# pecos/tps

Hardware: AMD Instinct MI355X
Metric: DG RHS evals/sec (MDOF/s) for 3D p=3 reacting cyl at 1/2/4/8 MI355X (higher is better)
Workload: dtype f64

## Files before the change

tps_amd/csrc/kernels.hpp:

```cpp
#ifndef TPSRHS_KERNELS_HPP_
#define TPSRHS_KERNELS_HPP_

#include <hip/hip_runtime.h>

#include <type_traits>

#include "basis.hpp"
#include "physics_dryair.hpp"

namespace tpsrhs {

#ifndef TPSRHS_NO_MFMA
#define TPSRHS_NO_MFMA 0
#endif
#ifndef TPSRHS_LEAN_GENERAL
#define TPSRHS_LEAN_GENERAL 0
#endif
constexpr int cmax(int a, int b) { return a > b ? a : b; }

#ifndef TPSRHS_STAMP
#define TPSRHS_STAMP 0
#endif
#if TPSRHS_STAMP
constexpr int NSTAMP = 16, STAMP_BLOCKS = 1 << 16;
// ... 92 lines not shown
  static constexpr int Q1 = ((DIM_ - 1) + 2 * P_) / 2 + 1 + NC_;
  static constexpr int QV = P_ + 1 + NC_;
  static constexpr int NQV = (DIM_ == 3) ? QV * QV * QV : QV * QV;
  static constexpr int NQ = (DIM_ == 3) ? Q1 * Q1 : Q1;
  static constexpr int NW = (DIM_ == 3) ? Q1 * N1 : 1;
  static constexpr int NFACES = 2 * DIM_;
  static constexpr int NV = 1 << DIM_;
  static constexpr int BLOCK = (NC_ && DIM_ == 3 && P_ >= 2) ? 128 : ((NPE <= 64) ? 64 : ((NPE <= 128) ? 128 : 256));
  static constexpr int EPB = (DIM_ == 3 && NC_) ? (P_ == 3 ? 1 : 2)
                             : (DIM_ == 3 && P_ == 1) ? 3
                             : (DIM_ == 2 && NC_ && P_ == 1) ? 10
                                                             : BLOCK / NPE;
  static constexpr int NODES = EPB * NPE;
  static constexpr int PF = 2 * EPB;
  static constexpr int TN = PF * NF;
  static constexpr int TW = PF * NW;
  static constexpr int TQ = PF * NQ;
  static constexpr int LN = EPB * NF;
  static constexpr int Q_ROUNDS = (TQ + BLOCK - 1) / BLOCK;
  static_assert(DIM_ == 2 || Q_ROUNDS == 1, "3-D: one round of face quadrature points per direction pair");
  static_assert(!(DIM_ == 2 && NC_) || Q_ROUNDS == 1, "2-D Gauss-Lobatto pair: one round per direction pair");
  static constexpr int TQ2 = 2 * TQ;
  static constexpr int Q2_ROUNDS = (TQ2 + BLOCK - 1) / BLOCK;
};

template <class PH, class = void>
struct lean_one_hex : std::false_type {};
template <class PH>
struct lean_one_hex<PH, std::enable_if_t<PH::LEAN_ONE_HEX>> : std::true_type {};
template <class C, class PH>
constexpr bool coulomb_tab() {
  return lean_one_hex<PH>::value && C::DIM == 3 && C::P == 3 && C::NC == 0;
}

template <class C>
struct Tab {
  double x[C::N1], w[C::N1], iw[C::N1], D[C::N1 * C::N1], b0[C::N1], b1[C::N1];
  double xq[C::Q1], wq[C::Q1], B[C::Q1 * C::N1];
  double xv[C::QV], wv[C::QV];
};

struct ForcingDev {
  int has_pg, nheat, nsponge, pad;
  double pg[3];
  struct Heat {
    double value, radius, len;
    double p1[3], axis[3];
  } heat[TPSRHS_MAXHEATSOURCES];
  struct Sponge {
    int type, pad;
    double normal[3], p0[3], pinit[3];
    double r1, r2, mult;
    double target[TPSRHS_MAXEQUATIONS];
    int mixed_out, n_plane;
    const int *plane_nodes;
    double *msum;
  } sponge[TPSRHS_MAXSPONGEZONES];
  const double *joule;
  int nps, pad2;
  struct Scalar {
    double x0[3], radius, value;
  } ps[TPSRHS_MAXPASSIVESCALARS];
};

struct RkDev {
  int mode, sp_first, sp_last, pad;
// ... 1408 lines not shown
      const double val = lean1_point<C>(Wb, k, bq, ll);
      if (k >= 1 && k <= NVEL)
        gv[(k - 1) + CD * DIM] = val;
      else if (CD == 0)
        gn[k] = 0.0 + n[CD] * val;
      else
        gn[k] += n[CD] * val;
    }
#pragma unroll
    for (int k = 0; k < NEQ; k++) {
      if (k >= 1 && k <= NVEL)
        asm volatile("" : "+v"(gv[(k - 1) + CD * DIM]));
      else
        asm volatile("" : "+v"(gn[k]));
    }
    block_sync<C::BLOCK>();
  };
  stage(std::integral_constant<int, 0>());
  stage(std::integral_constant<int, 1>());
  stage(std::integral_constant<int, 2>());
}
template <class C, class PH, int D>
__device__ inline void lean1_state_dir(const double *sU, double *Tb, double *Wb, const Tab<C> &tab, const Tables1D &ct0, double *u,
                                       const LeanLane<C> &ll) {
  const Tables1D &ct = fresh_table(ct0);
  lean1_lines<C, D, PH::NEQ>(sU, Tb, Wb, ct, ll, ll.template trace_src<D>());
  double bq[C::N1];
#pragma unroll
  for (int a = 0; a < C::N1; a++) bq[a] = tab.B[ll.pb + a];
#pragma unroll
  for (int k = 0; k < PH::NEQ; k++) u[k] = lean1_point<C>(Wb, k, bq, ll);
  block_sync<C::BLOCK>();
}
template <class C, class PH>
__device__ inline void visc_phase_lean1(const MeshDev &m, const int2 *sFI, typename PH::PRef prm0, int e0, const double *sU,
                                        const double *gradUp_q, bool node_on0, double *sJ, double *Tb, double *Wb,
                                        const double *sV, const Tab<C> &tab, const Tables1D &ct, double *__restrict__ TB,
                                        int tid0 STAMP_PARAM) {
  constexpr int NEQ = PH::NEQ, DIM = C::DIM;
  static_assert(DIM == 3 && C::Q_ROUNDS == 1 && PH::NVEL == 3 && C::BLOCK == 64 && C::EPB == 1, "3-D, one wave = one hex");
  const bool node_on = __builtin_amdgcn_readfirstlane(node_on0) != 0;
#pragma clang loop unroll(disable)
  for (int d = 0; d < DIM; d++) {
    typename PH::PRef prm = PH::relaunder(prm0);
    int tid = tid0;
    asm volatile("" : "+v"(tid));
    const int pf = tid / C::NQ, q = tid - pf * C::NQ;
    const int le = pf >> 1, s = pf & 1;
    const bool on = tid < C::TQ && (e0 + le) < m.ne;
    int nb = 0;
    double n[DIM] = {1.0, 0.0, 0.0};
    if (on) {
      double wq, Xq[DIM];
      nb = sFI[le * C::NFACES + 2 * d + s].x;
      face_geometry_rt<C>(d, &sV[le * C::NV * DIM], tab, s, q, n, wq, Xq);
    }
    const int np_lane = on ? PH::visc_passes(prm, nb) : 0;
    const int npass = (__ballot(np_lane == 2) != 0) ? 2 : ((__ballot(np_lane >= 1) != 0) ? 1 : 0);
    double *out = TB + static_cast<int64_t>((e0 + le) * C::NFACES + 2 * d + s) * ((NEQ - 1) * C::NQ) + q;
    if (on && np_lane == 0) {
#pragma unroll
      for (int eq = 1; eq < NEQ; eq++) out[(eq - 1) * C::NQ] = 0.0;
    }
#pragma clang loop unroll(disable)
    for (int pass = 0; pass < npass; pass++) {
      double u[NEQ];
      int tid1 = tid0;
      asm volatile("" : "+v"(tid1));
      const LeanLane<C> ll(static_cast<unsigned>(tid1) & (C::BLOCK - 1));
      if (d == 0)
        lean1_state_dir<C, PH, 0>(sU, Tb, Wb, tab, ct, u, ll);
      else if (d == 1)
        lean1_state_dir<C, PH, 1>(sU, Tb, Wb, tab, ct, u, ll);
      else
        lean1_state_dir<C, PH, 2>(sU, Tb, Wb, tab, ct, u, ll);
      STAMP(5);
      PH::clamp_species(u);
      double gnext[NEQ];
      unsigned long long ga = lean1_grad_base<C>(gradUp_q, e0);
      const unsigned long long gstep = static_cast<unsigned long long>(m.ndofs) * sizeof(double);
      if (node_on) {
        lean1_issue_grad<NEQ>(ga, gstep, ll.lane, gnext);
      } else {
#pragma unroll
        for (int eq = 0; eq < NEQ; eq++) gnext[eq] = 0.0;
      }
      typename PH::ViscLean cf;
      if (pass < np_lane) {
        typename PH::PRef pq = PH::relaunder(prm);
        double Us[NEQ];
        typename PH::WallFlux w;
        PH::visc_pass_state(pq, nb, pass, u, n, Us, w);
        if constexpr (coulomb_tab<C, PH>())
          PH::template visc_point_lean<true>(pq, Us, w, cf);
        else
          PH::visc_point_lean(pq, Us, w, cf);
      }
      STAMP(6);
      double gv[DIM * DIM], gn[NEQ];
      if (d == 0)
        lean1_grad_dir<C, PH, 0>(ga, gstep, node_on, gnext, sJ, Tb, Wb, tab, ct, n, gv, gn, ll);
      else if (d == 1)
        lean1_grad_dir<C, PH, 1>(ga, gstep, node_on, gnext, sJ, Tb, Wb, tab, ct, n, gv, gn, ll);
      else
        lean1_grad_dir<C, PH, 2>(ga, gstep, node_on, gnext, sJ, Tb, Wb, tab, ct, n, gv, gn, ll);
      STAMP(7);
      if (pass < np_lane) {
        double f[NEQ];
        PH::visc_normal_flux_lean(cf, gv, gn, n, f);
        if (nb >= 0) {
#pragma unroll
          for (int eq = 1; eq < NEQ; eq++) out[(eq - 1) * C::NQ] = f[eq];
        } else if (pass == 0) {
#pragma unroll
          for (int eq = 1; eq < NEQ; eq++) out[(eq - 1) * C::NQ] = -0.5 * f[eq];
        } else {
#pragma unroll
          for (int eq = 1; eq < NEQ; eq++) out[(eq - 1) * C::NQ] -= 0.5 * f[eq];
        }
      }
      STAMP(8);
    }
  }
}
template <class C, class PH>
__device__ inline void visc_phase_2d(const MeshDev &m, const int2 *sFI, typename PH::PRef prm, int e0,
// ... 209 lines not shown
  jump(std::integral_constant<int, 1>());
  if (DIM == 3) {
    trace_lines<C, (DIM == 3 ? 2 : 0), NEQ>(sUp, sJ, ct, tid);
    block_sync<C::BLOCK>();
    store_neighbour_traces<C, NEQ>(ta2, sJ, sJ + NEQ * C::TN, tid);
    block_sync<C::BLOCK>();
    jump(std::integral_constant<int, (DIM == 3 ? 2 : 0)>());
  }
  if constexpr (C::NC) {
    if constexpr (C::NPE == 64 && C::BLOCK == 128 && !TPSRHS_NO_MFMA) {
      static_assert(L::V >= 64 * 17, "LDS buffer of the MFMA inverse mass");
      nc_apply_minv_mfma<C, NEQ * DIM>(m.minv, pool + L::O_V, node_on, e0, nd, tid, g);
    }
    else
      nc_apply_minv<C, NEQ * DIM>(m.minv, pool + L::O_V, node_on, e0 + le_n, le_n, nd, tid, g);
  }

  STAMP(3);
  if (node_on) {
    const unsigned n = static_cast<unsigned>(e0 + le_n) * C::NPE + nd;
#pragma unroll
    for (int k = 0; k < NEQ * DIM; k++) field_ptr(gradUp, k, m.ndofs)[n] = g[k];
    if constexpr (L::G_IN_LDS) {
#pragma unroll
      for (int k = 0; k < NEQ * DIM; k++) sJ[k * C::NODES + tid] = g[k];
    }
  }
  if (L::G_IN_LDS) block_sync<C::BLOCK>();
  STAMP(4);
  if constexpr (L::LEAN3D) {
    asm volatile("s_waitcnt vmcnt(0)" ::: "memory");
    const double *gq = gradUp;
    const unsigned node = static_cast<unsigned>(e0 + le_n) * C::NPE + nd;
    if constexpr (PH::LEAN_ONE_HEX && C::EPB == 1 && C::BLOCK % C::LN == 0 && !TPSRHS_LEAN_GENERAL)
      visc_phase_lean1<C, PH>(m, sFI, prm, e0, sU, gq, node_on, sJ, sUp, sW, sV, tab, ct, TB, tid STAMP_ARG);
    else
      visc_phase_lean3d<C, PH>(m, sFI, prm, e0, sU, gq, node_on, node, sJ, sUp, sW, sV, tab, ct, TB, tid STAMP_ARG);
    STAMP_FLUSH();
    return;
  }

  if constexpr (DIM == 2) {
    if constexpr (PH::HEAVY) {
      __shared__ double sDist[C::NODES];
      const bool ml_on = m.ml.distance != nullptr;
      if (ml_on) {
        if (tid < C::NODES)
          sDist[tid] = node_on ? m.ml.distance[static_cast<int64_t>(e0 + le_n) * C::NPE + nd] : 0.0;
        block_sync<C::BLOCK>();
      }
      visc_phase_2d<C, PH>(m, sFI, prm, e0, sU, g, node_on, sJ, sUp, sV, tab, ct, TB, tid, ml_on ? sDist : nullptr);
    } else {
      visc_phase_2d<C, PH>(m, sFI, prm, e0, sU, g, node_on, sJ, sUp, sV, tab, ct, TB, tid);
    }
  } else if constexpr (PH::TWO_STEP && C::Q_ROUNDS == 1) {
    visc_phase_heavy3d<C, PH>(m, sFI, prm, e0, sU, sJ, sUp, sW, sV, tab, ct, TB, tid STAMP_ARG);
  } else if constexpr (PH::HEAVY) {
#pragma clang loop unroll(disable)
    for (int d = 0; d < DIM; d++) {
      double v[C::Q_ROUNDS][L::NVF];
      if (d == 0)
        visc_interp_dir<C, PH, 0>(sU, g, node_on, sJ, sUp, sW, tab, ct, v, tid);
      else if (d == 1)
        visc_interp_dir<C, PH, 1>(sU, g, node_on, sJ, sUp, sW, tab, ct, v, tid);
      else
        visc_interp_dir<C, PH, (DIM == 3 ? 2 : 0)>(sU, g, node_on, sJ, sUp, sW, tab, ct, v, tid);
      visc_points<C, PH>(m, sFI, prm, e0, d, v, sV, tab, TB, tid);
    }
  } else {
// ... 573 lines not shown
  }
  if (node_on) {
#pragma unroll
    for (int eq = 0; eq < NEQ; eq++) sU[eq * C::NODES + tid] = u[eq];
  }
  block_sync<C::BLOCK>();
  FSTAMP(1);

  double inv_mass = 0.0, speed = 0.0;
  double src[NEQ];
#pragma unroll
  for (int eq = 0; eq < NEQ; eq++) src[eq] = 0.0;
  if (node_on) {
    double F[NEQ * DIM];
    double radius = 1.0;
    double Xn[DIM] = {};
    if constexpr (PH::AXISYM || (PH::HEAVY && DIM == 2)) {
      if (PH::AXISYM || m.vs.enabled) {
        double xi[DIM];
#pragma unroll
        for (int d = 0; d < DIM; d++) xi[d] = tab.x[idx[d]];
        position<DIM>(&sV[le_n * C::NV * DIM], xi, Xn);
      }
      if (PH::AXISYM) radius = Xn[0];
    }
    {
      double uc[NEQ];
#pragma unroll
      for (int eq = 0; eq < NEQ; eq++) uc[eq] = u[eq];
      PH::clamp_species(uc);
      const typename PH::State st = PH::make_state(prm, uc);
      speed = PH::max_char_speed(prm, uc, st);
      typename PH::FluxCoef fc;
      if constexpr (coulomb_tab<C, PH>())
        PH::template flux_coeffs<true>(prm, uc, st, fc);
      else if constexpr (PH::TWO_STEP)
        PH::flux_coeffs(prm, uc, st, fc);
      if (PH::HAS_SOURCE) {
        double up[NEQ];
        PH::prim(prm, u, up);
        PH::source(prm, u, up, gr, src);
        if constexpr (PH::AXISYM) PH::axisym_source(prm, u, up, gr, radius, src);
      }

      if constexpr (PH::HEAVY && DIM == 2) {
        const bool ml_on = m.ml.distance != nullptr;
        __shared__ double sVsw[C::BLOCK];
        const EddyCtx ec = closure_ctx(m, true, ml_on ? m.ml.distance[static_cast<int64_t>(e0 + le_n) * C::NPE + nd] : 0.0, Xn, sVsw);
        if constexpr (PH::TWO_STEP)
          PH::total_flux(prm, uc, st, fc, gr, PH::AXISYM ? radius : -1.0, F, ec);
        else
          PH::total_flux(prm, uc, st, gr, radius, F, ec);
      } else if constexpr (PH::TWO_STEP)
        PH::total_flux(prm, uc, st, fc, gr, PH::AXISYM ? radius : -1.0, F);
      else if constexpr (PH::AXISYM)
        PH::total_flux(prm, uc, st, gr, radius, F);
      else if constexpr (PH::LES) {
        PointCtx pc;
        double xn[DIM];
#pragma unroll
        for (int d = 0; d < DIM; d++) xn[d] = tab.x[idx[d]];
        position<DIM>(&sV[le_n * C::NV * DIM], xn, pc.X);
        pc.delta = prm.elem_delta[e0 + le_n];
        PH::total_flux(prm, uc, st, gr, F, &pc);
      } else
        PH::total_flux(prm, uc, st, gr, F);
    }
// ... 323 lines not shown
```

tps_amd/csrc/physics_plasma.hpp:

```cpp
#ifndef TPSRHS_PHYSICS_PLASMA_HPP_
#define TPSRHS_PHYSICS_PLASMA_HPP_

#include <hip/hip_runtime.h>

#include "physics_dryair.hpp"
#if __has_include("coulomb_table.hpp")
#include "coulomb_table.hpp"
#define TPSRHS_HAVE_COULOMB_TABLE 1
#endif

namespace tpsrhs {

#pragma clang fp reciprocal(on)

constexpr double kRgas = 8.3144598;
constexpr double kAvogadro = 6.0221409e+23;
constexpr double kBoltz = kRgas / kAvogadro;
constexpr double kEps0 = 8.8541878128e-12;
constexpr double kQe = 1.60218e-19;
constexpr double kMolarQe = kQe * kAvogadro;
constexpr double kPi = 3.14159265358979323846;
constexpr double kXeps = 1.0e-30;

struct TableDev {
// ... 3 lines not shown
};
struct ChemDev {
  int num_reactions, electron_index;
  double min_temperature;
  double energy[TPSRHS_MAXREACTIONS];
  double rate[TPSRHS_MAXCHEMPARAMS * TPSRHS_MAXREACTIONS];
  double keq[TPSRHS_MAXCHEMPARAMS * TPSRHS_MAXREACTIONS];
  signed char reactant[TPSRHS_MAXSPECIES * TPSRHS_MAXREACTIONS];
  signed char product[TPSRHS_MAXSPECIES * TPSRHS_MAXREACTIONS];
  signed char model[TPSRHS_MAXREACTIONS];
  signed char detailed_balance[TPSRHS_MAXREACTIONS];
  TableDev table[TPSRHS_MAXREACTIONS];
  signed char table_share[TPSRHS_MAXREACTIONS];
  int radiation;
  TableDev nec;
};

constexpr int PLASMA_MAXBC = 8;
template <int NSP>
struct PlasmaParams {
  double mw[NSP], charge[NSP], eform[NSP], cv[NSP], cp[NSP];
  double imw[NSP], mwp[NSP], sq_mwp[NSP], kf_imwp[NSP], sq_muw_idfc[NSP * NSP];
  double vf_sq_mwp[NSP], ke_fac, ke_fac3, qkb_charge[NSP], rg_imw[NSP], icv_e;
  double c_visc, c_bulk, c_k, c_ke, c_diff[NSP], c_mtfreq[NSP];
  int c_eidx;
  int third_order, multiply;
  int coll[NSP * NSP];
  int cmask_diag, cmask_e, cmask_h;
  double mult_flux[4], mult_spcs, mult_diff, mult_mobil;
  const ChemDev *chem;
  int eq_system, use_bc_in_grad, num_bcs, axisymmetric;
  BcDev bc[PLASMA_MAXBC];
  const double *ctab;
};

__device__ inline double ipow(double x, int k) {
  double r = 1.0;
  for (int i = 0; i < k; i++) r *= x;
  return r;
}
template <class TD>
__device__ inline int table_interval(const TD &t, double xe) {
  if (t.inv_dx > 0.0) {
    int g = static_cast<int>((xe - t.x0) * t.inv_dx);
    g = max(0, min(t.n - 2, g));
    if (g > 0 && !(xe > t.x[g])) g--;
    if (g < t.n - 2 && xe > t.x[g + 1]) g++;
    if ((g == 0 || xe > t.x[g]) && (g == t.n - 2 || !(xe > t.x[g + 1]))) return g;
  }
  int count = t.n, first = 0;
  while (count > 0) {
    int it = first;
    const int step = count / 2;
    it += step;
    if (xe > t.x[it]) {
      first = ++it;
      count -= step + 1;
    } else {
      count = step;
    }
  }
  first = max(1, min(t.n - 1, first));
  return first - 1;
}
template <class TD>
__device__ inline double table_eval(const TD &t, double xe) {
// ... 82 lines not shown
  for (int r = 0; r < NUNI; r++) {
    if (todo) {
      const int u = __builtin_amdgcn_readfirstlane(idx);
      if (idx == u) {
        coulomb::horner<NF>(ctab + u * coulomb::STRIDE, t, g);
        todo = false;
      }
    }
  }
  if (todo) coulomb::horner<NF>(tab + idx * coulomb::STRIDE, t, g);
}
template <int NF>
__device__ inline void cfit_tab(const double *tab, const Arg &a, double (&out)[NF]) {
  static_assert(NF == 2 || NF == 8, "att11 and rep22, or all eight");
  const bool on = tab != nullptr && coulomb::in_range(a.ln);
  if (on) {
    ctab_eval<NF, TPSRHS_COULOMB_UNIFORM>(tab, a.ln, true, out);
#pragma unroll
    for (int f = 0; f < NF; f++) out[f] *= a.inv2;
  } else if constexpr (NF == 8) {
    double A[4], B[4];
    cfit_n<4>(kFitA, a, A);
    cfit_n<4>(kFitB, a, B);
#pragma unroll
    for (int f = 0; f < 4; f++) {
      out[f] = A[f];
      out[4 + f] = B[f];
    }
  } else {
    out[0] = att11(a);
    out[1] = rep22(a);
  }
}
#endif
__constant__ static double c_coulomb[2][2][5][4] = {
    {{{0.2150, 5.2194, 1.0472, 1.2435}, {0.0991, 7.4684, 1.0155, 1.1536}, {0.0616, 7.8271, 0.9452, 1.1105},
      {0.0308, 13.9567, 0.9511, 1.1803}, {0.0232, 13.7888, 0.9148, 1.1532}},
     {{0, 0, 0, 0}, {0.2423, 4.6796, 1.3290, 1.1279}, {0.1221, 8.7542, 1.3875, 1.1110}, {0.0619, 18.2538, 1.4341, 1.1618},
      {0, 0, 0, 0}}},
    {{{0.3904, 0.9100, 1.1025, 1.0544}, {0.1547, 1.6597, 1.1725, 0.9792}, {0.0814, 2.5815, 1.1948, 0.9570},
      {0.0683, 1.9774, 1.2033, 0.8264}, {0.0346, 4.5177, 1.2132, 0.9294}},
     {{0, 0, 0, 0}, {0.4128, 1.2436, 1.1830, 1.0123}, {0.2203, 1.8832, 1.2059, 0.9851}, {0.1323, 2.7248, 1.2129, 0.9847},
      {0, 0, 0, 0}}}};
__device__ inline double ArAr11(double lnT) { return 2.2910e-18 * fexp(-0.3032 * lnT); }
__device__ inline double ArAr22(double T) { return 1.7e-18 * fast_rsqrt(fast_sqrt(T)); }
__device__ inline double iArAr22(double sqrtT) { return fast_sqrt(sqrtT) * (1.0 / 1.7e-18); }
__device__ inline double ArAr1P11(double lnT) { return 4.574321e-18 * fexp(-0.1805 * lnT); }
__device__ inline double eAr1r(int r, double logT) {
  const double C[5][9] = {
      {6.36254140e-18, 1.84835040e-18, -5.87727093e-18, 3.20023027e-18, -8.50509054e-19, 1.28163820e-19,
       -1.11712910e-20, 5.25649382e-22, -1.03296658e-23},
      {1.91338172e-17, 5.45418129e-18, -1.78361685e-17, 9.75657946e-18, -2.61115722e-18, 3.98310268e-19,
       -3.53503678e-20, 1.70375066e-21, -3.45211955e-23},
      {3.04685398e-17, 8.39750994e-18, -2.88132528e-17, 1.60147037e-17, -4.34837891e-18, 6.73136845e-19,
       -6.06704580e-20, 2.97216168e-21, -6.12760944e-23},
      {3.90777949e-17, 1.04696956e-17, -3.73774204e-17, 2.10610498e-17, -5.79029566e-18, 9.07573157e-19,
       -8.28466766e-20, 4.11188110e-21, -8.59225098e-23},
      {4.41333290e-17, 1.15696010e-17, -4.25651305e-17, 2.42442440e-17, -6.73359258e-18, 1.06641697e-18,
       -9.83933863e-20, 4.93775812e-21, -1.04362372e-22}};
  double fit = C[r - 1][0] * fast_rcp(logT), pw = 1.0;
#pragma unroll
  for (int k = 1; k < 9; k++) {
    fit += C[r - 1][k] * pw;
    pw *= logT;
  }
  return fit;
// ... 24 lines not shown
  }
}
}

#ifndef TPSRHS_PLASMA_MINW_FLUX
#define TPSRHS_PLASMA_MINW_FLUX 2
#endif
#ifndef TPSRHS_PLASMA_MINW_GRAD3
#define TPSRHS_PLASMA_MINW_GRAD3 2
#endif
#ifndef TPSRHS_PLASMA_MINW_GRAD_LEAN
#define TPSRHS_PLASMA_MINW_GRAD_LEAN 3
#endif
enum { TRANSPORT_CONSTANT = 0, TRANSPORT_ARGON_MINIMAL = 1, TRANSPORT_ARGON_MIXTURE = 2 };

template <int DIM_, int NVEL_, int NSP_, bool AMBI, bool TWOT, int TRANSPORT>
struct PlasmaPhys {
  static constexpr int DIM = DIM_, NVEL = NVEL_, NSP = NSP_;
  static constexpr int NACTIVE = AMBI ? NSP_ - 2 : NSP_ - 1;
  static constexpr int NEQ = NVEL_ + 2 + NACTIVE + (TWOT ? 1 : 0);
  static constexpr int IE = NSP_ - 2, IB = NSP_ - 1;
  static constexpr int ITH = NVEL_ + 1, ITE = NEQ - 1;
  static constexpr bool HAS_SOURCE = true;
  static constexpr bool TWO_TEMPERATURE = TWOT;
  static constexpr int MAX_ORDER = 4;
  static constexpr bool HAS_NR_BC = false;
  static constexpr bool LES = false;
  static constexpr bool HAS_MIXED_OUT = false;
  static constexpr bool VISC_USES_GRAD_RHO = true;
  static constexpr bool AXISYM = NVEL_ > DIM_;
  static constexpr int MINW_GRAD = (NSP_ > 3) ? 1 : TPSRHS_PLASMA_MINW_GRAD3;
  static constexpr bool LEAN_TRACE = (NSP_ == 3) && (DIM_ == 3);
  static constexpr bool LEAN_ONE_HEX = LEAN_TRACE && !TWOT && TRANSPORT == TRANSPORT_ARGON_MINIMAL;
  static constexpr bool LAUNDER_FLUX = false;
  static constexpr int minw_grad(int dim, int p, int nc) {
    return (LEAN_TRACE && dim == 3 && !nc && p <= 3) ? TPSRHS_PLASMA_MINW_GRAD_LEAN : MINW_GRAD;
  }
  static constexpr int MINW_FLUX = (NSP_ > 6 || (NSP_ > 3 && DIM_ == 3)) ? 1 : TPSRHS_PLASMA_MINW_FLUX;
  typedef PlasmaParams<NSP_> Params;
  typedef const Params *KArg;
  typedef const Params __attribute__((address_space(4))) &PRef;
  typedef const BcDev __attribute__((address_space(4))) &BcRef;
  __device__ static inline PRef pref(KArg k) { return *(const Params __attribute__((address_space(4))) *)k; }
  __device__ static inline PRef relaunder(PRef p) {
    const unsigned long long a = reinterpret_cast<unsigned long long>(&p);
    unsigned lo = __builtin_amdgcn_readfirstlane(static_cast<unsigned>(a));
    unsigned hi = __builtin_amdgcn_readfirstlane(static_cast<unsigned>(a >> 32));
    asm volatile("" : "+s"(lo), "+s"(hi));
    return *reinterpret_cast<const Params __attribute__((address_space(4))) *>((static_cast<unsigned long long>(hi) << 32) | lo);
  }
  struct Transport {};

  struct State {
    double ir, k, p, pe, Th, Te, c;
    double vel[NVEL];
    double n[NSP];
  };

  __device__ static inline void number_densities(PRef p, const double *U, double *n) {
#pragma unroll
    for (int sp = 0; sp < NSP; sp++) n[sp] = 0.0;
#pragma unroll
    for (int sp = 0; sp < NACTIVE; sp++) n[sp] = U[NVEL + 2 + sp] * p.imw[sp];
    double rhoB = U[0];
#pragma unroll
    for (int sp = 0; sp < NACTIVE; sp++) rhoB -= p.mw[sp] * n[sp];
// ... 215 lines not shown
    double att, rep, ar1p, are, arar;
  };
  template <int L, int R>
  __device__ static inline CollTab coll_table(int mask, bool with_e, const MixColl &c) {
    CollTab t;
    t.att = t.rep = t.ar1p = t.are = t.arar = 0.0;
    const coll::Arg &a = with_e ? c.e : c.h;
    const double ln = with_e ? c.lnTe : c.lnTh;
    if (mask & (1 << TPSRHS_CLMB_ATT)) {
      const double *k = coll::c_coulomb[0][L - 1][R - 1];
      t.att = c.circle * coll::cfit(k[0], k[1], k[2], k[3], a);
    }
    if (mask & (1 << TPSRHS_CLMB_REP)) {
      const double *k = coll::c_coulomb[1][L - 1][R - 1];
      t.rep = c.circle * coll::cfit(k[0], k[1], k[2], k[3], a);
    }
    if (mask & (1 << TPSRHS_AR_AR1P)) t.ar1p = coll::ArAr1P11(ln);
    if (mask & (1 << TPSRHS_AR_E)) t.are = coll::eAr1r(R, ln);
    if (mask & (1 << TPSRHS_AR_AR)) t.arar = (L == 1) ? coll::ArAr11(ln) : coll::ArAr22(c.Th);
    return t;
  }
  __device__ static inline double coll_pick(PRef p, int i, int j, const CollTab &t) {
    const int a = i < j ? i : j, b = i < j ? j : i;
    const int type = p.coll[a + b * NSP];
    const double q_att = t.att, q_rep = t.rep, q_ar1p = t.ar1p, q_are = t.are, q_arar = t.arar;
    double v = q_arar;
    v = (type == TPSRHS_AR_E) ? q_are : v;
    v = (type == TPSRHS_AR_AR1P) ? q_ar1p : v;
    v = (type == TPSRHS_CLMB_REP) ? q_rep : v;
    v = (type == TPSRHS_CLMB_ATT) ? q_att : v;
    return v;
  }

  template <bool CTAB = false>
  __device__ static inline void transport_coeffs(PRef p, const double *U, double Th, double Te, bool diffusion,
                                                 TCoef &t) {
#ifndef TPSRHS_HAVE_COULOMB_TABLE
    static_assert(!CTAB, "coulomb_table.hpp is not part of this build");
#endif
    static_assert(!CTAB || (!TWOT && TRANSPORT == TRANSPORT_ARGON_MINIMAL), "the table serves the single-temperature argon-minimal closure");
    const Species q = species(p, U);
#pragma unroll
    for (int sp = 0; sp < NSP; sp++) {
      t.n[sp] = q.n[sp];
      t.Y[sp] = q.Y[sp];
      t.dX[sp] = t.mob[sp] = 0.0;
    }
    t.intot = q.intot;
    t.imho = 0.0;
    double diff[NSP] = {}, mob[NSP] = {};
    const double iTe = fast_rcp(Te), iTh = TWOT ? fast_rcp(Th) : iTe;
    if (TRANSPORT == TRANSPORT_CONSTANT) {
      t.visc = p.c_visc;
      t.bulk = p.c_bulk;
      t.k = p.c_k;
      t.ke = p.c_ke;
#pragma unroll
      for (int sp = 0; sp < NSP; sp++) {
        diff[sp] = p.c_diff[sp];
        const double itemp = (sp == p.c_eidx) ? iTe : iTh;
        mob[sp] = p.qkb_charge[sp] * itemp * diff[sp];
      }
    } else if (TRANSPORT == TRANSPORT_ARGON_MIXTURE) {
      const MixColl c = mix_inputs(p, q.n, Th, Te);
      const double sTe = fast_sqrt(Te), sTh = TWOT ? fast_sqrt(Th) : sTe;
      t.visc = t.bulk = t.k = 0.0;
      {
        const CollTab d22 = coll_table<2, 2>(p.cmask_diag, false, c);
#pragma unroll
        for (int sp = 0; sp < NSP; sp++) {
          if (sp == IE) continue;
          const double sv = p.vf_sq_mwp[sp] * sTh * fast_rcp(coll_pick(p, sp, sp, d22));
// ... 39 lines not shown
            ibd[i + j * NSP] = ibd[j + i * NSP] = ((i == IE || j == IE) ? nrsTe : nrsTh) * p.sq_muw_idfc[i + j * NSP] *
                                                  coll_pick(p, i, j, (i == IE || j == IE) ? pe : ph);
#pragma unroll
        for (int i = 0; i < NSP; i++) {
          double a = 0.0;
#pragma unroll
          for (int j = 0; j < NSP; j++)
            if (i != j) a += (q.X[j] + kXeps) * ibd[i + j * NSP];
          diff[i] = (1.0 - q.Y[i]) * fast_rcp(a);
          mob[i] = p.qkb_charge[i] * ((i == IE) ? iTe : iTh) * diff[i];
        }
      }
      if (p.multiply) {
        t.visc *= p.mult_flux[0];
        t.bulk *= p.mult_flux[1];
        t.k *= p.mult_flux[2];
        t.ke *= p.mult_flux[3];
#pragma unroll
        for (int sp = 0; sp < NSP; sp++) {
          diff[sp] *= p.mult_diff;
          mob[sp] *= p.mult_mobil;
        }
      }
    } else {
      const double sTe = fast_sqrt(Te), sTh = TWOT ? fast_sqrt(Th) : sTe;
      const Debye d = debye(q.n, Th, Te, iTh, iTe);
      const double lnTe = flog(Te), lnTh = TWOT ? flog(Th) : lnTe;
      double QeAr, Qatt, rep22h;
      if (p.third_order) {
        double A[4], B[4], QN[5];
#ifdef TPSRHS_HAVE_COULOMB_TABLE
        if constexpr (CTAB) {
          double g[8];
          coll::cfit_tab<8>(p.ctab, d.e, g);
#pragma unroll
          for (int f = 0; f < 4; f++) {
            A[f] = g[f];
            B[f] = g[4 + f];
          }
        } else
#endif
        {
          coll::cfit_n<4>(coll::kFitA, d.e, A);
          coll::cfit_n<4>(coll::kFitB, d.e, B);
        }
        coll::eAr1r_n<5>(lnTe, QN);
        Qatt = A[0] * d.circle;
        QeAr = QN[0];
        const double Q2[3] = {d.circle * A[1], d.circle * A[2], d.circle * A[3]};
        const double QI[5] = {Qatt, d.circle * B[0], d.circle * B[1], d.circle * B[2], d.circle * B[3]};
        rep22h = TWOT ? coll::rep22(d.h) * d.circle : Q2[0];
        t.ke = third_order_ke(q.X, Q2, QI, QN, sTe, p.ke_fac3);
      } else {
        QeAr = coll::eAr1r(1, lnTe);
#ifdef TPSRHS_HAVE_COULOMB_TABLE
        if constexpr (CTAB) {
          double g[2];
          coll::cfit_tab<2>(p.ctab, d.e, g);
          Qatt = g[0] * d.circle;
          rep22h = g[1] * d.circle;
        } else
#endif
        {
          Qatt = coll::att11(d.e) * d.circle;
          rep22h = coll::rep22(d.h) * d.circle;
        }
        t.ke = p.ke_fac * sTe * q.X[I_E] * fast_rcp(TWOT ? coll::rep22(d.e) * d.circle : rep22h);
      }
      const double sv_ion = p.vf_sq_mwp[I_ION] * sTh * fast_rcp(rep22h);
      const double sv_n = p.vf_sq_mwp[I_N] * sTh * coll::iArAr22(sTh);
      t.bulk = 0.0;
      t.visc = q.X[I_ION] * sv_ion + q.X[I_N] * sv_n;
      t.k = q.X[I_ION] * (sv_ion * p.kf_imwp[I_ION]) + q.X[I_N] * (sv_n * p.kf_imwp[I_N]);
      __builtin_amdgcn_sched_barrier(0);
      if (diffusion) {
        const double nrsTe = q.ntot * (sTe * iTe), nrsTh = TWOT ? q.ntot * (sTh * iTh) : nrsTe;
        double ibd[NSP * NSP];
#pragma unroll
        for (int i = 0; i < NSP * NSP; i++) ibd[i] = 0.0;
        ibd[I_E + I_N * NSP] = ibd[I_N + I_E * NSP] = nrsTe * p.sq_muw_idfc[I_E + I_N * NSP] * QeAr;
        ibd[I_N + I_ION * NSP] = ibd[I_ION + I_N * NSP] = nrsTh * p.sq_muw_idfc[I_N + I_ION * NSP] * coll::ArAr1P11(lnTh);
        ibd[I_E + I_ION * NSP] = ibd[I_ION + I_E * NSP] = nrsTe * p.sq_muw_idfc[I_E + I_ION * NSP] * Qatt;
#pragma unroll
        for (int i = 0; i < NSP; i++) {
          double a = 0.0;
#pragma unroll
          for (int j = 0; j < NSP; j++)
            if (i != j) a += (q.X[j] + kXeps) * ibd[i + j * NSP];
          diff[i] = (1.0 - q.Y[i]) * fast_rcp(a);
          mob[i] = p.qkb_charge[i] * ((i == I_E) ? iTe : iTh) * diff[i];
        }
// ... 178 lines not shown
#pragma unroll
    for (int i = 0; i < DIM; i++) divV += g[(1 + i) + i * NEQ];
    double tau_t[DIM] = {};
    if (AXISYM) {
      if (radius > 0) divV += s.vel[0] / radius;
      double ttr = g[3 + 0 * NEQ];
      if (radius > 0) ttr -= s.vel[2] / radius;
      tau_t[0] = ttr * t.visc;
      tau_t[1] = t.visc * g[3 + 1 * NEQ];
    }
#pragma unroll
    for (int i = 0; i < DIM; i++) {
      double vt = 0.0;
#pragma unroll
      for (int j = 0; j < DIM; j++) {
        double st = t.visc * (g[(1 + j) + i * NEQ] + g[(1 + i) + j * NEQ]);
        if (i == j) st += bulk * divV;
        Fv[(1 + j) + i * NEQ] = st;
        vt += st * s.vel[j];
      }
      if (AXISYM) {
        Fv[(1 + 2) + i * NEQ] = tau_t[i];
        vt += s.vel[2] * tau_t[i];
      }
      double e = vt + k * g[ITH + i * NEQ];
#pragma unroll
      for (int sp = 0; sp < NSP; sp++) e -= h[sp] * t.V[sp + i * NSP];
      Fv[ITH + i * NEQ] += e;
#pragma unroll
      for (int sp = 0; sp < NACTIVE; sp++) Fv[(NVEL + 2 + sp) + i * NEQ] = -U[NVEL + 2 + sp] * t.V[sp + i * NSP];
    }
  }
  typedef TCoef FluxCoef;
  template <bool CTAB = false>
  __device__ static inline void flux_coeffs(PRef p, const double *U, const State &s, FluxCoef &c) {
    if (p.eq_system == TPSRHS_EULER) return;
    transport_coeffs<CTAB>(p, U, s.Th, s.Te, true, c);
  }
  __device__ static inline void total_flux(PRef p, const double *U, const State &s, const FluxCoef &c,
                                           const double *g, double radius, double *F, const EddyCtx &ec = eddy_off()) {
    double Fv[NEQ * DIM];
    visc_flux(p, U, s, c, g, radius, Fv, ec);
    const double H = U[ITH] + s.p;
#pragma unroll
    for (int d = 0; d < DIM; d++) {
      F[0 + d * NEQ] = U[1 + d] - Fv[0 + d * NEQ];
#pragma unroll
      for (int i = 0; i < NVEL; i++) F[1 + i + d * NEQ] = U[1 + i] * s.vel[d] + (i == d ? s.p : 0.0) - Fv[1 + i + d * NEQ];
      F[ITH + d * NEQ] = s.vel[d] * H - Fv[ITH + d * NEQ];
#pragma unroll
      for (int sp = 0; sp < NACTIVE; sp++)
        F[(NVEL + 2 + sp) + d * NEQ] = U[NVEL + 2 + sp] * s.vel[d] - Fv[(NVEL + 2 + sp) + d * NEQ];
      if (TWOT) F[ITE + d * NEQ] = (U[ITE] + s.pe) * s.vel[d] - Fv[ITE + d * NEQ];
    }
  }
  struct WallFlux {
    bool species, heavy_heat, electron_heat;
    double Vn[NSP], hf, ef, nm;
  };
  __device__ static inline WallFlux no_prescription() {
    WallFlux w;
    w.species = w.heavy_heat = w.electron_heat = false;
#pragma unroll
    for (int sp = 0; sp < NSP; sp++) w.Vn[sp] = 0.0;
    w.hf = w.ef = 0.0;
    w.nm = 1.0;
    return w;
  }
  __device__ static inline void visc_normal_flux(PRef p, const double *U, const double *g, const double *n,
                                                 double radius, const WallFlux &w, double *Fn, const EddyCtx &ec = eddy_off()) {
// ... 324 lines not shown
      Fn[1 + i] = sn;
      e += sn * c.vel[i];
    }
    double HF = 0.0, EF = 0.0;
    if (w.heavy_heat) {
      HF = w.hf * w.nm;
    } else {
      const double k = TWOT ? c.t.k : c.t.k + c.t.ke;
      HF -= k * gn[ITH];
#pragma unroll
      for (int sp = 0; sp < NSP; sp++)
        if (!(TWOT && sp == IE)) HF += c.h[sp] * Vn[sp];
    }
    if (TWOT) {
      if (w.electron_heat) {
        EF = w.ef * w.nm;
      } else {
        EF -= c.t.ke * gn[ITE];
        EF += c.h[IE] * Vn[IE];
      }
    }
    Fn[ITH] = e - HF - EF;
#pragma unroll
    for (int sp = 0; sp < NACTIVE; sp++) Fn[NVEL + 2 + sp] = -U[NVEL + 2 + sp] * Vn[sp];
    if (TWOT) Fn[ITE] = -EF;
  }
  static constexpr int NIN = 1 + NACTIVE;
  struct ViscLean {
    double mu, bulkp, kq, ke;
    double vel[NVEL];
    double hf0, ef0, sf0[NACTIVE];
    double hfc[NIN], efc[NIN], sfc[NACTIVE][NIN];
  };
  template <bool CTAB = false>
  __device__ static inline void visc_point_lean(PRef p, const double *U, const WallFlux &w, ViscLean &L) {
    const State s = make_state(p, U);
    TCoef t;
    transport_coeffs<CTAB>(p, U, s.Th, s.Te, !w.species, t);
    double h[NSP];
    enthalpies(p, s, h);
    L.mu = t.visc;
    L.bulkp = t.bulk - 2. / 3. * t.visc;
#pragma unroll
    for (int d = 0; d < NVEL; d++) L.vel[d] = s.vel[d];
    L.kq = w.heavy_heat ? 0.0 : (TWOT ? t.k : t.k + t.ke);
    L.hf0 = w.heavy_heat ? w.hf * w.nm : 0.0;
    L.ke = (TWOT && !w.electron_heat) ? t.ke : 0.0;
    L.ef0 = (TWOT && w.electron_heat) ? w.ef * w.nm : 0.0;
#pragma unroll
    for (int sp = 0; sp < NACTIVE; sp++) L.sf0[sp] = 0.0;
#pragma unroll
    for (int j = 0; j < NIN; j++) {
      L.hfc[j] = L.efc[j] = 0.0;
#pragma unroll
      for (int sp = 0; sp < NACTIVE; sp++) L.sfc[sp][j] = 0.0;
    }
    if (w.species) {
      double Vn[NSP];
#pragma unroll
      for (int sp = 0; sp < NSP; sp++) Vn[sp] = w.Vn[sp] * w.nm;
      if (!w.heavy_heat) {
#pragma unroll
        for (int sp = 0; sp < NSP; sp++)
          if (!(TWOT && sp == IE)) L.hf0 += h[sp] * Vn[sp];
      }
      if (TWOT && !w.electron_heat) L.ef0 += h[IE] * Vn[IE];
#pragma unroll
      for (int sp = 0; sp < NACTIVE; sp++) L.sf0[sp] = -U[NVEL + 2 + sp] * Vn[sp];
    } else {
#pragma unroll
      for (int j = 0; j < NIN; j++) {
// ... 373 lines not shown
```

tps_amd/csrc/tpsrhs.hip:

```cpp
#include "operator.hpp"
#include "element_geometry.hpp"
#include "integrals.hpp"
#include "locate_device.hpp"
#include "operator_plan.hpp"
#include "physics_dryair.hpp"
#include "physics_dryair_axisym.hpp"
#include "physics_plasma.hpp"
#include "plasma_params_host.hpp"
#include "point_locate.hpp"
#include "record_log.hpp"
#include "sampling.hpp"
#include "statistics.hpp"
#include "time_integrators.hpp"
#include "wall_distance.hpp"
#include "wall_faces.hpp"

#include <dlfcn.h>

#include <cmath>
#include <map>
#include <mutex>
#include <new>
#include <thread>
#include <type_traits>
// ... 68 lines not shown
    std::vector<double> t(coulomb::SIZE);
    coll::coulomb_table_fill(t.data());
    return t;
  }();
  return table;
}

template <int NSP>
void fill_plasma_params(tpsrhs_operator *op, const tpsrhs_disc *disc, const tpsrhs_physics *phys, int num_bcs,
                        const tpsrhs_bc *bcs) {
  static_assert(sizeof(PlasmaParams<NSP>) <= sizeof(op->params), "parameter block too large");
  PlasmaParams<NSP> &p = *new (op->params) PlasmaParams<NSP>;
  std::unique_ptr<ChemDev> c(new ChemDev);
  try {
    tpsrhs::fill_plasma_params<NSP>(p, *c, disc, phys, num_bcs, bcs, [op](const tpsrhs_table &t) { return upload_table(op, t); });
  } catch (const UnsupportedConfig &e) {
    throw Unsupported(e.what());
  }
  op->d_chem = DevBuf<ChemDev>(1);
  p.chem = static_cast<ChemDev *>(op->d_chem.get());
  HIP_CHECK(hipMemcpy(op->d_chem.get(), c.get(), sizeof(ChemDev), hipMemcpyHostToDevice));
}

void fill_mixture_params(tpsrhs_operator *op, const OperatorPlan &pl, const tpsrhs_disc *disc, const tpsrhs_physics *phys,
                         int num_bcs, const tpsrhs_bc *bcs) {
  switch (phys->mixture.num_species) {
    case 3:
      fill_plasma_params<3>(op, disc, phys, num_bcs, bcs);
      if (pl.coulomb_table) {
        const char *env = std::getenv("TPSRHS_COULOMB_TABLE");
        if (!env || env[0] != '0') {
          op->d_coulomb = DevBuf<double>(coulomb_table_host());
          reinterpret_cast<PlasmaParams<3> *>(op->params)->ctab = op->d_coulomb.get();
        }
      }
      break;
    case 4: fill_plasma_params<4>(op, disc, phys, num_bcs, bcs); break;
    case 5: fill_plasma_params<5>(op, disc, phys, num_bcs, bcs); break;
    case 6: fill_plasma_params<6>(op, disc, phys, num_bcs, bcs); break;
    case 7: fill_plasma_params<7>(op, disc, phys, num_bcs, bcs); break;
    default: fill_plasma_params<8>(op, disc, phys, num_bcs, bcs); break;
  }
  char msg[512] = {0};
  const int rc = load_family(pl.unit)(op, phys->mixture.two_temperature ? 1 : 0, pl.transport, msg, static_cast<int>(sizeof msg));
  if (rc == TPSRHS_ERR_UNSUPPORTED) throw Unsupported(msg);
  if (rc == TPSRHS_ERR_INVALID_ARGUMENT) throw std::invalid_argument(msg);
  if (rc != TPSRHS_OK) throw DeviceError(msg);
}

void upload_lte_tables(tpsrhs_operator *op, LteParams *lp, const tpsrhs_physics *phys) {
  const tpsrhs_lte &in = phys->lte;
  lp->tab_e = upload_table(op, in.energy_table);
  lp->tab_R = upload_table(op, in.gas_constant_table);
  lp->tab_c = upload_table(op, in.sound_speed_table);
  tpsrhs_table rev = in.energy_table;
  rev.x_data = in.energy_table.f_data;
  rev.f_data = in.energy_table.x_data;
  lp->tab_T = upload_table(op, rev);
  {
    const int N = in.energy_table.n_data, nh = 4 * (N - 1);
    const double *ex = in.energy_table.f_data;
    const double de = (ex[N - 1] - ex[0]) / nh;
    std::vector<int> hint(nh);
    int idx = 0;
    for (int j = 0; j < nh; j++) {
      const double left = ex[0] + j * de;
// ... 851 lines not shown
int tpsrhs_math_eval(int function, int64_t n, const double *x, double *y) {
  if (function < 0 || function > 6 || n < 0 || !x || !y) return fail(TPSRHS_ERR_INVALID_ARGUMENT, "math_eval");
  return guarded([&] {
    int ndev = 0;
    if (hipGetDeviceCount(&ndev) != hipSuccess || ndev == 0) throw std::runtime_error("no HIP device visible");
    if (n > 0) {
      hipLaunchKernelGGL(k_math_eval, dim3(static_cast<unsigned>((n + 255) / 256)), dim3(256), 0, nullptr, function, n, x, y);
      HIP_CHECK(hipGetLastError());
    }
    HIP_CHECK(hipDeviceSynchronize());
  });
}

namespace {
__global__ void k_coulomb_eval(int route, const double *tab, int64_t n, const double *__restrict__ x, double *__restrict__ out) {
  const int64_t i = static_cast<int64_t>(blockIdx.x) * 256 + threadIdx.x;
  if (i >= n) return;
  coll::Arg a;
  a.ln = x[i];
  a.inv2 = 1.0;
  double g[8];
  if (route == 0 || !coulomb::in_range(a.ln)) {
    coll::cfit_tab<8>(nullptr, a, g);
  } else if (route == 1) {
    coll::ctab_eval<8, 2>(tab, a.ln, true, g);
  } else {
    coll::ctab_eval<8, 0>(tab, a.ln, true, g);
  }
#pragma unroll
  for (int f = 0; f < 8; f++) out[f * n + i] = g[f];
}
}

int tpsrhs_coulomb_eval(int route, int64_t n, const double *x, double *out) {
  if (route < 0 || route > 2 || n < 0 || !x || !out) return fail(TPSRHS_ERR_INVALID_ARGUMENT, "coulomb_eval");
  return guarded([&] {
    int ndev = 0;
    if (hipGetDeviceCount(&ndev) != hipSuccess || ndev == 0) throw std::runtime_error("no HIP device visible");
    DevBuf<double> tab(coulomb_table_host());
    if (n > 0) {
      hipLaunchKernelGGL(k_coulomb_eval, dim3(static_cast<unsigned>((n + 255) / 256)), dim3(256), 0, nullptr, route, tab.get(), n, x, out);
      HIP_CHECK(hipGetLastError());
    }
    HIP_CHECK(hipDeviceSynchronize());
  });
}

int tpsrhs_table_eval(const tpsrhs_table *table, int64_t n, const double *x, double *f) {
  if (!table || n < 0 || !x || !f) return fail(TPSRHS_ERR_INVALID_ARGUMENT, "table_eval");
  return guarded([&] {
    int ndev = 0;
    if (hipGetDeviceCount(&ndev) != hipSuccess || ndev == 0) throw std::runtime_error("no HIP device visible");
    tpsrhs_operator tmp;
    (void)hipGetDevice(&tmp.device);
    const TableDev td = upload_table(&tmp, *table);
    if (n > 0) {
      hipLaunchKernelGGL(k_table_eval, dim3(static_cast<unsigned>((n + 255) / 256)), dim3(256), 0, nullptr, td, n, x, f);
      HIP_CHECK(hipGetLastError());
    }
    HIP_CHECK(hipDeviceSynchronize());
  });
}

int tpsrhs_mult_times(tpsrhs_handle h, int capacity, double *milliseconds) {
  if (!h || h->sets_recorded == 0 || !milliseconds) return 0;
  if (hipStreamSynchronize(h->stream) != hipSuccess) return 0;
  const int nsets = static_cast<int>(std::min<int64_t>(h->sets_recorded, tpsrhs_operator::MAXSETS));
  int n = 0;
  for (; n < nsets && n < capacity; n++) {
    float ms = 0.f;
    if (hipEventElapsedTime(&ms, h->evs[n][0], h->evs[n][NKERN]) != hipSuccess) return n;
    milliseconds[n] = ms;
  }
// ... 950 lines not shown
```

Before: 13170.

## Stage Coulomb table intervals in a per-wave LDS window for transport evaluation

```diff
diff --git a/tps_amd/csrc/coulomb_probe.hip b/tps_amd/csrc/coulomb_probe.hip
--- /dev/null
+++ b/tps_amd/csrc/coulomb_probe.hip
@@ -0,0 +1,36 @@
+#include <hip/hip_runtime.h>
+
+#include <algorithm>
+#include <cstdint>
+
+#include "physics_plasma.hpp"
+
+using namespace tpsrhs;
+
+namespace {
+constexpr int COULOMB_PROBE_BLOCKS = 4;
+__global__ __launch_bounds__(64) void k_coulomb_eval_window(const double *tab, int64_t n, const double *__restrict__ x,
+                                                            double *__restrict__ out) {
+  typedef coll::Window<TPSRHS_COULOMB_WINDOW_W> Win;
+  __shared__ __attribute__((aligned(16))) double mem[Win::DOUBLES];
+  Win win;
+  win.create(mem, true);
+  for (int64_t c0 = static_cast<int64_t>(blockIdx.x) * 64; c0 < n; c0 += static_cast<int64_t>(gridDim.x) * 64) {
+    const int64_t i = c0 + threadIdx.x;
+    if (i < n) {
+      coll::Arg a;
+      a.ln = x[i];
+      a.inv2 = 1.0;
+      double g[8];
+      coll::cfit_tab<8>(tab, a, g, win);
+#pragma unroll
+      for (int f = 0; f < 8; f++) out[f * n + i] = g[f];
+    }
+  }
+}
+}
+
+void coulomb_probe_window(const double *tab, int64_t n, const double *x, double *out) {
+  hipLaunchKernelGGL(k_coulomb_eval_window, dim3(static_cast<unsigned>(std::min<int64_t>((n + 63) / 64, COULOMB_PROBE_BLOCKS))),
+                     dim3(64), 0, nullptr, tab, n, x, out);
+}
diff --git a/tps_amd/csrc/kernels.hpp b/tps_amd/csrc/kernels.hpp
--- a/tps_amd/csrc/kernels.hpp
+++ b/tps_amd/csrc/kernels.hpp
@@ -148,6 +148,28 @@
 constexpr bool coulomb_tab() {
   return lean_one_hex<PH>::value && C::DIM == 3 && C::P == 3 && C::NC == 0;
 }
+#ifndef TPSRHS_COULOMB_WINDOW_GRAD
+#define TPSRHS_COULOMB_WINDOW_GRAD 4
+#endif
+#ifndef TPSRHS_COULOMB_WINDOW_GRAD_POOL
+#define TPSRHS_COULOMB_WINDOW_GRAD_POOL 1
+#endif
+#ifndef TPSRHS_COULOMB_WINDOW_FLUX
+#define TPSRHS_COULOMB_WINDOW_FLUX 3
+#endif
+struct NoCoulombWindow {};
+template <class C, class PH, int W, bool ON_ = coulomb_tab<C, PH>() && (W > 0)>
+struct CoulombWin {
+  static constexpr bool ON = false;
+  typedef NoCoulombWindow type;
+};
+template <class C, class PH, int W>
+struct CoulombWin<C, PH, W, true> {
+  static_assert(C::BLOCK == 64, "the window belongs to ONE wave: no workgroup barrier orders its loads and reads");
+  static constexpr bool ON = true;
+  typedef typename PH::template CoulombWindow<W> type;
+  static constexpr int DOUBLES = type::DOUBLES;
+};
 
 template <class C>
 struct Tab {
@@ -1622,11 +1644,11 @@
   for (int k = 0; k < PH::NEQ; k++) u[k] = lean1_point<C>(Wb, k, bq, ll);
   block_sync<C::BLOCK>();
 }
-template <class C, class PH>
+template <class C, class PH, class CWIN>
 __device__ inline void visc_phase_lean1(const MeshDev &m, const int2 *sFI, typename PH::PRef prm0, int e0, const double *sU,
                                         const double *gradUp_q, bool node_on0, double *sJ, double *Tb, double *Wb,
                                         const double *sV, const Tab<C> &tab, const Tables1D &ct, double *__restrict__ TB,
-                                        int tid0 STAMP_PARAM) {
+                                        int tid0, const CWIN &win STAMP_PARAM) {
   constexpr int NEQ = PH::NEQ, DIM = C::DIM;
   static_assert(DIM == 3 && C::Q_ROUNDS == 1 && PH::NVEL == 3 && C::BLOCK == 64 && C::EPB == 1, "3-D, one wave = one hex");
   const bool node_on = __builtin_amdgcn_readfirstlane(node_on0) != 0;
@@ -1681,7 +1703,11 @@
         double Us[NEQ];
         typename PH::WallFlux w;
         PH::visc_pass_state(pq, nb, pass, u, n, Us, w);
-        if constexpr (coulomb_tab<C, PH>())
+        if constexpr (!std::is_same<CWIN, NoCoulombWindow>::value) {
+          if constexpr (TPSRHS_COULOMB_WINDOW_GRAD_POOL) win.clear();
+          PH::template visc_point_lean<true>(pq, Us, w, cf, win);
+        }
+        else if constexpr (coulomb_tab<C, PH>())
           PH::template visc_point_lean<true>(pq, Us, w, cf);
         else
           PH::visc_point_lean(pq, Us, w, cf);
@@ -1957,9 +1983,18 @@
     asm volatile("s_waitcnt vmcnt(0)" ::: "memory");
     const double *gq = gradUp;
     const unsigned node = static_cast<unsigned>(e0 + le_n) * C::NPE + nd;
-    if constexpr (PH::LEAN_ONE_HEX && C::EPB == 1 && C::BLOCK % C::LN == 0 && !TPSRHS_LEAN_GENERAL)
-      visc_phase_lean1<C, PH>(m, sFI, prm, e0, sU, gq, node_on, sJ, sUp, sW, sV, tab, ct, TB, tid STAMP_ARG);
-    else
+    if constexpr (PH::LEAN_ONE_HEX && C::EPB == 1 && C::BLOCK % C::LN == 0 && !TPSRHS_LEAN_GENERAL) {
+      typedef CoulombWin<C, PH, TPSRHS_COULOMB_WINDOW_GRAD> CW;
+      typename CW::type win;
+      if constexpr (CW::ON && TPSRHS_COULOMB_WINDOW_GRAD_POOL) {
+        static_assert(CW::DOUBLES <= L::SUP, "the window takes the T chunk of the pool");
+        win.create(sUp, prm.cwin != 0);
+      } else if constexpr (CW::ON) {
+        __shared__ __attribute__((aligned(16))) double sCw[CW::DOUBLES];
+        win.create(sCw, prm.cwin != 0);
+      }
+      visc_phase_lean1<C, PH>(m, sFI, prm, e0, sU, gq, node_on, sJ, sUp, sW, sV, tab, ct, TB, tid, win STAMP_ARG);
+    } else
       visc_phase_lean3d<C, PH>(m, sFI, prm, e0, sU, gq, node_on, node, sJ, sUp, sW, sV, tab, ct, TB, tid STAMP_ARG);
     STAMP_FLUSH();
     return;
@@ -2599,7 +2634,13 @@
       const typename PH::State st = PH::make_state(prm, uc);
       speed = PH::max_char_speed(prm, uc, st);
       typename PH::FluxCoef fc;
-      if constexpr (coulomb_tab<C, PH>())
+      if constexpr (CoulombWin<C, PH, TPSRHS_COULOMB_WINDOW_FLUX>::ON) {
+        typedef CoulombWin<C, PH, TPSRHS_COULOMB_WINDOW_FLUX> CW;
+        __shared__ __attribute__((aligned(16))) double sCw[CW::DOUBLES];
+        typename CW::type win;
+        win.create(sCw, prm.cwin != 0);
+        PH::template flux_coeffs<true>(prm, uc, st, fc, win);
+      } else if constexpr (coulomb_tab<C, PH>())
         PH::template flux_coeffs<true>(prm, uc, st, fc);
       else if constexpr (PH::TWO_STEP)
         PH::flux_coeffs(prm, uc, st, fc);
diff --git a/tps_amd/csrc/physics_plasma.hpp b/tps_amd/csrc/physics_plasma.hpp
--- a/tps_amd/csrc/physics_plasma.hpp
+++ b/tps_amd/csrc/physics_plasma.hpp
@@ -59,6 +59,7 @@
   int eq_system, use_bc_in_grad, num_bcs, axisymmetric;
   BcDev bc[PLASMA_MAXBC];
   const double *ctab;
+  int cwin;
 };
 
 __device__ inline double ipow(double x, int k) {
@@ -207,6 +208,82 @@
     out[1] = rep22(a);
   }
 }
+#if defined(__HIPCC__)
+#ifndef TPSRHS_COULOMB_WINDOW_W
+#define TPSRHS_COULOMB_WINDOW_W 2
+#endif
+__device__ inline void wave_fence() {
+  __builtin_amdgcn_fence(__ATOMIC_RELEASE, "wavefront");
+  __builtin_amdgcn_wave_barrier();
+  __builtin_amdgcn_fence(__ATOMIC_ACQUIRE, "wavefront");
+}
+template <int W_>
+struct Window {
+  static_assert(W_ >= 1 && W_ <= coulomb::NI, "intervals of the table");
+  static constexpr int W = W_;
+  static constexpr int COEF = W_ * coulomb::STRIDE;
+  static constexpr int DOUBLES = COEF + 2;
+  typedef double __attribute__((address_space(3))) *Lds;
+  Lds lds;
+  bool on;
+  __device__ inline void create(double *mem, bool enabled) {
+    lds = (Lds)mem;
+    on = enabled;
+    clear();
+  }
+  __device__ inline void clear() const {
+    wave_fence();
+    *reinterpret_cast<int __attribute__((address_space(3))) *>(lds + COEF) = -2 * coulomb::NI;
+    wave_fence();
+  }
+};
+template <int NF, class WIN>
+__device__ inline void ctab_window_eval(const WIN &win, const double *tab, double x, double (&g)[NF]) {
+  const int idx = coulomb::interval(x);
+  const double t = coulomb::local(x, idx);
+  int rel = -1;
+  if (win.on) {
+    const unsigned long long act = __ballot(1);
+    int lo = __builtin_amdgcn_readfirstlane(idx);
+    for (;;) {
+      const unsigned long long below = __ballot(idx < lo);
+      if (below == 0) break;
+      lo = __builtin_amdgcn_readlane(idx, static_cast<int>(__builtin_ctzll(below)));
+    }
+    int __attribute__((address_space(3))) *bp = reinterpret_cast<int __attribute__((address_space(3))) *>(win.lds + WIN::COEF);
+    wave_fence();
+    int base = __builtin_amdgcn_readfirstlane(*bp);
+    if (lo < base || lo >= base + WIN::W) {
+      base = lo < coulomb::NI - WIN::W ? lo : coulomb::NI - WIN::W;
+      const int rank = static_cast<int>(__builtin_amdgcn_mbcnt_hi(static_cast<unsigned>(act >> 32),
+                                                                  __builtin_amdgcn_mbcnt_lo(static_cast<unsigned>(act), 0u)));
+      const int step = __builtin_popcountll(act);
+      typedef double __attribute__((ext_vector_type(2))) d2;
+      const d2 *src = reinterpret_cast<const d2 *>(tab + base * coulomb::STRIDE);
+      d2 __attribute__((address_space(3))) *dst = reinterpret_cast<d2 __attribute__((address_space(3))) *>(win.lds);
+      for (int pc = rank; pc < WIN::COEF / 2; pc += step) dst[pc] = src[pc];
+      if (rank == 0) *bp = base;
+      wave_fence();
+    }
+    rel = idx - base;
+  }
+  if (rel >= 0 && rel < WIN::W)
+    coulomb::horner<NF>(static_cast<const double __attribute__((address_space(3))) *>(win.lds) + rel * coulomb::STRIDE, t, g);
+  else
+    coulomb::horner<NF>(tab + idx * coulomb::STRIDE, t, g);
+}
+template <int NF, class WIN>
+__device__ inline void cfit_tab(const double *tab, const Arg &a, double (&out)[NF], const WIN &win) {
+  static_assert(TPSRHS_COULOMB_UNIFORM == 0, "the window replaces the per-lane route");
+  if (tab != nullptr && coulomb::in_range(a.ln)) {
+    ctab_window_eval<NF>(win, tab, a.ln, out);
+#pragma unroll
+    for (int f = 0; f < NF; f++) out[f] *= a.inv2;
+  } else {
+    cfit_tab<NF>(nullptr, a, out);
+  }
+}
+#endif
 #endif
 __constant__ static double c_coulomb[2][2][5][4] = {
     {{{0.2150, 5.2194, 1.0472, 1.2435}, {0.0991, 7.4684, 1.0155, 1.1536}, {0.0616, 7.8271, 0.9452, 1.1105},
@@ -297,6 +374,10 @@
   static constexpr int MINW_GRAD = (NSP_ > 3) ? 1 : TPSRHS_PLASMA_MINW_GRAD3;
   static constexpr bool LEAN_TRACE = (NSP_ == 3) && (DIM_ == 3);
   static constexpr bool LEAN_ONE_HEX = LEAN_TRACE && !TWOT && TRANSPORT == TRANSPORT_ARGON_MINIMAL;
+#if defined(TPSRHS_HAVE_COULOMB_TABLE) && defined(__HIPCC__)
+  template <int W>
+  using CoulombWindow = coll::Window<W>;
+#endif
   static constexpr bool LAUNDER_FLUX = false;
   static constexpr int minw_grad(int dim, int p, int nc) {
     return (LEAN_TRACE && dim == 3 && !nc && p <= 3) ? TPSRHS_PLASMA_MINW_GRAD_LEAN : MINW_GRAD;
@@ -578,12 +659,13 @@
     return v;
   }
 
-  template <bool CTAB = false>
+  template <bool CTAB = false, class... WIN>
   __device__ static inline void transport_coeffs(PRef p, const double *U, double Th, double Te, bool diffusion,
-                                                 TCoef &t) {
+                                                 TCoef &t, const WIN &...win) {
 #ifndef TPSRHS_HAVE_COULOMB_TABLE
     static_assert(!CTAB, "coulomb_table.hpp is not part of this build");
 #endif
+    static_assert(sizeof...(WIN) <= (CTAB ? 1 : 0), "at most one window, and only of the table");
     static_assert(!CTAB || (!TWOT && TRANSPORT == TRANSPORT_ARGON_MINIMAL), "the table serves the single-temperature argon-minimal closure");
     const Species q = species(p, U);
 #pragma unroll
@@ -689,7 +771,7 @@
 #ifdef TPSRHS_HAVE_COULOMB_TABLE
         if constexpr (CTAB) {
           double g[8];
-          coll::cfit_tab<8>(p.ctab, d.e, g);
+          coll::cfit_tab<8>(p.ctab, d.e, g, win...);
 #pragma unroll
           for (int f = 0; f < 4; f++) {
             A[f] = g[f];
@@ -713,7 +795,7 @@
 #ifdef TPSRHS_HAVE_COULOMB_TABLE
         if constexpr (CTAB) {
           double g[2];
-          coll::cfit_tab<2>(p.ctab, d.e, g);
+          coll::cfit_tab<2>(p.ctab, d.e, g, win...);
           Qatt = g[0] * d.circle;
           rep22h = g[1] * d.circle;
         } else
@@ -958,10 +1040,10 @@
     }
   }
   typedef TCoef FluxCoef;
-  template <bool CTAB = false>
-  __device__ static inline void flux_coeffs(PRef p, const double *U, const State &s, FluxCoef &c) {
+  template <bool CTAB = false, class... WIN>
+  __device__ static inline void flux_coeffs(PRef p, const double *U, const State &s, FluxCoef &c, const WIN &...win) {
     if (p.eq_system == TPSRHS_EULER) return;
-    transport_coeffs<CTAB>(p, U, s.Th, s.Te, true, c);
+    transport_coeffs<CTAB>(p, U, s.Th, s.Te, true, c, win...);
   }
   __device__ static inline void total_flux(PRef p, const double *U, const State &s, const FluxCoef &c,
                                            const double *g, double radius, double *F, const EddyCtx &ec = eddy_off()) {
@@ -1352,11 +1434,11 @@
     double hf0, ef0, sf0[NACTIVE];
     double hfc[NIN], efc[NIN], sfc[NACTIVE][NIN];
   };
-  template <bool CTAB = false>
-  __device__ static inline void visc_point_lean(PRef p, const double *U, const WallFlux &w, ViscLean &L) {
+  template <bool CTAB = false, class... WIN>
+  __device__ static inline void visc_point_lean(PRef p, const double *U, const WallFlux &w, ViscLean &L, const WIN &...win) {
     const State s = make_state(p, U);
     TCoef t;
-    transport_coeffs<CTAB>(p, U, s.Th, s.Te, !w.species, t);
+    transport_coeffs<CTAB>(p, U, s.Th, s.Te, !w.species, t, win...);
     double h[NSP];
     enthalpies(p, s, h);
     L.mu = t.visc;
diff --git a/tps_amd/csrc/tpsrhs.hip b/tps_amd/csrc/tpsrhs.hip
--- a/tps_amd/csrc/tpsrhs.hip
+++ b/tps_amd/csrc/tpsrhs.hip
@@ -124,6 +124,8 @@
         if (!env || env[0] != '0') {
           op->d_coulomb = DevBuf<double>(coulomb_table_host());
           reinterpret_cast<PlasmaParams<3> *>(op->params)->ctab = op->d_coulomb.get();
+          const char *win = std::getenv("TPSRHS_COULOMB_WINDOW");
+          reinterpret_cast<PlasmaParams<3> *>(op->params)->cwin = (!win || win[0] != '0') ? 1 : 0;
         }
       }
       break;
@@ -1041,13 +1043,18 @@
 }
 }
 
+extern "C++" void coulomb_probe_window(const double *tab, int64_t n, const double *x, double *out);
+
 int tpsrhs_coulomb_eval(int route, int64_t n, const double *x, double *out) {
-  if (route < 0 || route > 2 || n < 0 || !x || !out) return fail(TPSRHS_ERR_INVALID_ARGUMENT, "coulomb_eval");
+  if (route < 0 || route > 3 || n < 0 || !x || !out) return fail(TPSRHS_ERR_INVALID_ARGUMENT, "coulomb_eval");
   return guarded([&] {
     int ndev = 0;
     if (hipGetDeviceCount(&ndev) != hipSuccess || ndev == 0) throw std::runtime_error("no HIP device visible");
     DevBuf<double> tab(coulomb_table_host());
-    if (n > 0) {
+    if (n > 0 && route == 3) {
+      coulomb_probe_window(tab.get(), n, x, out);
+      HIP_CHECK(hipGetLastError());
+    } else if (n > 0) {
       hipLaunchKernelGGL(k_coulomb_eval, dim3(static_cast<unsigned>((n + 255) / 256)), dim3(256), 0, nullptr, route, tab.get(), n, x, out);
       HIP_CHECK(hipGetLastError());
     }
```

New measurement: 13890, median of 6. 1.05x the previous value.
